# elizabethfong/SparkSmithWaterman

Hardware: AMD Instinct MI355X
Metric: GCUPS (higher is better)
Workload: dtype int32

## Files before the change

### sparksmithwaterman_amd/csrc/swmi_ctx.cpp

```cpp
#include <cstdarg>
#include <cstdio>
#include <cstdlib>

#include "swmi_host.h"
#include "swmi_launch.h"

static thread_local std::string g_err;

int swmi_host::fail(int code, const char *fmt, ...) {
    char buf[512];
    va_list ap;
    va_start(ap, fmt);
    vsnprintf(buf, sizeof buf, fmt, ap);
    va_end(ap);
    g_err = buf;
    return code;
}

int swmi_io_fail(int code, const std::string &msg) { return fail(code, "%s", msg.c_str()); }

extern "C" int swmi_abi_version(void) { return SWMI_ABI_VERSION; }

extern "C" const char *swmi_last_error(void) { return g_err.c_str(); }

// ... 108 lines not shown
    } else if (!strcmp(name, "resident")) {
        if (value < -1 || value > 1) return fail(SWMI_ERR_INVALID, "resident must be -1 (automatic), 0 or 1");
        ctx->resident = (int)value;
    } else if (!strcmp(name, "scores_only")) {
        ctx->scores_only = value != 0;
    } else if (!strcmp(name, "stream_keep_records")) {
        ctx->stream_keep_records = value != 0;
    } else if (!strcmp(name, "device_strings")) {
        ctx->device_strings = value != 0;
    } else if (!strcmp(name, "tb_split")) {
        if (value < -1 || value > 1) return fail(SWMI_ERR_INVALID, "tb_split must be -1 (automatic), 0 or 1");
        ctx->tb_split = (int)value;
    } else if (!strcmp(name, "col_chunks")) {
        if (value < 0 || value > 4096) return fail(SWMI_ERR_INVALID, "col_chunks out of range");
        ctx->col_chunks = (uint32_t)value;
    } else if (!strcmp(name, "zero_copy")) {
        ctx->zero_copy = value != 0;
    } else if (!strcmp(name, "profiling")) {
        if (value < 0 || value > 2) return fail(SWMI_ERR_INVALID, "profiling must be 0, 1 (every stage) or 2 (the sweep only)");
        ctx->profiling = (int)value;
    } else if (!strcmp(name, "gap_open")) {
        if (value > 0) return fail(SWMI_ERR_INVALID, "gap_open must be <= 0 (a penalty), got %lld", (long long)value);
        if (value < INT32_MIN) return fail(SWMI_ERR_INVALID, "gap_open out of range");
        ctx->gap_open = (int32_t)value;
    } else if (!strcmp(name, "affine")) {
        if (value != -1 && value != 1) return fail(SWMI_ERR_INVALID, "affine must be -1 (when gap_open != 0) or 1 (always)");
        ctx->affine = (int)value;
    } else if (!strcmp(name, "align_mode")) {
        if (value != SWMI_ALIGN_LOCAL && value != SWMI_ALIGN_FIT && value != SWMI_ALIGN_GLOBAL)
            return fail(SWMI_ERR_INVALID, "align_mode must be 0 (local), 1 (fit) or 2 (global), got %lld", (long long)value);
// ... 347 lines not shown
```

### sparksmithwaterman_amd/csrc/swmi_device.h

```cpp
#pragma once
#include <stdint.h>

#if defined(__HIPCC__)
#define SWMI_HD __host__ __device__
#else
#define SWMI_HD
#endif

#define SWMI_SEQ_PAD_WORDS 24u
#define SWMI_RMAX          4
#ifndef SWMI_CK_BLOCKS
#define SWMI_CK_BLOCKS     2u
#endif
#define SWMI_CODE_PAD      0x1FFu

#define SWMI_LDS_BYTES (160u * 1024u)
#define SWMI_EMIT_SCRATCH_WORDS 128u
#define SWMI_TB_BLOCKS 16u
#define SWMI_TB_REFWIN_WORDS 96u
#define SWMI_RES_CELL_CAP 128u

#define SWMI_DIR_D 0u
#define SWMI_DIR_I 1u
#define SWMI_DIR_A 2u
// ... 18 lines not shown
    uint32_t read_id;
    uint32_t out_id;
    uint32_t pad;
    uint64_t dir_off;
    uint64_t seam_off;
};

#define SWMI_PAD_COLS 0x80000000u
#define SWMI_PAD_RESIDENT 0x40000000u

struct ColItem {
    uint32_t pair;
    uint32_t col0;
    uint32_t g_lo, g_hi;
};

struct StripItem {
    uint32_t pair, strip;
    uint32_t col0, g_lo, g_hi;
    uint32_t prog;
    uint32_t priv_stride;
    uint32_t pad;
    uint64_t priv_off;
};

struct PairOut {
    int32_t  score;
    uint32_t flags;
    uint64_t n_cells;
};
// ... 232 lines not shown
```

### sparksmithwaterman_amd/csrc/swmi_host.h

```cpp
#pragma once
#include <hip/hip_runtime.h>

#include <algorithm>
#include <atomic>
#include <condition_variable>
#include <cstdint>
#include <cstring>
#include <memory>
#include <mutex>
#include <string>
#include <thread>
#include <type_traits>
#include <unordered_map>
#include <vector>

#include "../../include/swmi.h"
#include "swmi_device.h"
#include "swmi_io_internal.h"

namespace swmi_host __attribute__((visibility("hidden"))) {
int fail(int code, const char *fmt, ...);
int check_offsets(const uint64_t *off, uint32_t n, const char *what);
int upload_device(swmi_ctx *ctx, swmi_batch *b, hipStream_t st, const uint8_t *ref_src, const uint8_t *read_src);
int settle_raw(swmi_batch *b);
// ... 129 lines not shown
    uint64_t arena_words_per_pair = 160;
    uint64_t arena_copy_wpp = 160;
    uint64_t recs_per_pair_x16 = 32;
    hipEvent_t ev[6] = {nullptr, nullptr, nullptr, nullptr, nullptr, nullptr};
    PinnedBuf h_err;
    DevBuf d_hdr_ring;
    uint32_t hdr_next = 0;
    DevBuf d_lut;
    DevBuf d_comp;
    int64_t spin_us = 2000;
    uint32_t dbg_strip_spins = 0;
    uint32_t dbg_reverse_strips = 0;
    uint32_t dbg_async_delay_us = 0;
    uint32_t auto_ties_x100 = 300;
    uint32_t col_chunks = 0;
    int tb_split = -1;
    bool ext_events = false;
    int tfused = -1;
    int resident = -1;
    int scores_only = 0;
    int stream_keep_records = 1;
    int device_strings = 1;
    bool cell_cap_set = false;
    int32_t gap_open = 0;
    int affine = -1;
    RunModes modes;
    std::mutex mat_mu;
    std::shared_ptr<const ScoreMatrix> matrix;
    std::thread worker;
    std::mutex job_mu;
// ... 33 lines not shown

struct Work {
    uint32_t pair;
    uint64_t cells;
    uint64_t dir_words;
    uint64_t seam_words;
};

struct __attribute__((visibility("hidden"))) PlanKey {
    bool valid = false;
    size_t lo = 0, hi = 0;
    const void *work = nullptr;
    swmi_params params{};
    uint32_t eff_mode = 0;
    uint32_t col_chunks = 0;
    bool reverse_strips = false;
    int resident = -1, tfused = -1;
    bool exact = false;
    bool scores_only = false;
    uint64_t mat_gen = 0;
    RunModes modes;
    const void *d_pairs = nullptr;
    size_t pairs_bytes = 0;
    bool operator==(const PlanKey &o) const {
        return valid == o.valid && lo == o.lo && hi == o.hi && work == o.work && memcmp(&params, &o.params, sizeof(swmi_params)) == 0 &&
               eff_mode == o.eff_mode && col_chunks == o.col_chunks && reverse_strips == o.reverse_strips && resident == o.resident &&
               tfused == o.tfused && exact == o.exact && scores_only == o.scores_only && mat_gen == o.mat_gen &&
               modes == o.modes && d_pairs == o.d_pairs && pairs_bytes == o.pairs_bytes;
    }
};

struct __attribute__((visibility("hidden"))) ChunkPlan {
    uint64_t dir_words = 0, seam_words = 0;
    uint64_t seam_priv_words = 0;
    uint32_t max_path = 0, max_read = 0;
    size_t n_strip_items = 0;
    size_t n_strip_chunks = 0;
    size_t n_col_items = 0;
    uint64_t n_windows = 0;
    size_t n_res = 0;
    uint32_t res_lds_words = 0, res_ops_words = 0;
    size_t n_tf = 0;
    uint32_t tf_max_m = 0, tf_max_n = 0, tf_max_path = 0;
    uint32_t aff_r_min = 0xFFFFFFFFu, aff_r_max = 0;
    size_t aff_n_long = 0;
};

struct swmi_batch {
    uint32_t n_refs = 0, n_reads = 0;
    bool paired = false;
    uint32_t n_src_refs = 0, n_src_reads = 0;
    std::vector<swmi_pair_spec> specs;
    bool sources_on_device = false;
// ... 98 lines not shown
```

### sparksmithwaterman_amd/csrc/swmi_plan.h

```cpp
#pragma once
#include <chrono>
#include <cstdlib>

#include "swmi_host.h"

using Clock = std::chrono::steady_clock;
static inline double us_between(Clock::time_point a, Clock::time_point c) { return std::chrono::duration<double, std::micro>(c - a).count(); }

static uint64_t path_bound(uint64_t n_, uint64_t m_, const swmi_params &p, int32_t smax, int align_mode = 0) {
    uint64_t path = n_ + m_;
    if (align_mode != 0) return path;
    if (smax > 0 && p.gap < 0 && p.mismatch <= smax) {
        const uint64_t g = (uint64_t)(-(int64_t)p.gap), mt = (uint64_t)smax;
        path = std::min(path, std::min(m_ + std::min(n_, mt * m_ / g), n_ + std::min(m_, mt * n_ / g)));
    }
    return path;
}

static uint64_t traceback_lds_bytes(uint32_t mode, uint64_t max_path, uint64_t max_read) {
    const uint64_t lds_words = (max_path + 3) / 4 + 1, lds_read_words = (max_read + 3) / 4 + 1;
    const uint64_t win = (uint64_t)SWMI_RMAX * 64;
    const uint64_t tile_words = mode == 0 ? 4ull * SWMI_TB_BLOCKS * win : (mode == 1 ? 32 + 8ull * SWMI_CK_BLOCKS * win : 4ull * SWMI_CK_BLOCKS * win);
    return 4ull * (tile_words + 4ull * (lds_words + lds_read_words + SWMI_TB_REFWIN_WORDS));
}
// ... 32 lines not shown
    if (c.g_hi < n_ck && (uint64_t)c.g_hi * CK_STEP_W > n) c.g_hi = n_ck;
    const int64_t c0 = (int64_t)g_lo * CK_STEP_W - 64 - (int64_t)span - 1;
    c.col0 = g_lo == 0 || c0 <= 0 ? 0u : (uint32_t)(c0 / CK_STEP_W * CK_STEP_W);
    return c;
}

struct Planner {
    const swmi_ctx *ctx;
    const swmi_batch *b;
    const swmi_params &P;
    size_t np;
    ChunkPlan &plan;
    PlanItems &it;
    bool cols_possible = false;
    uint64_t chunk_budget = 1;
    bool res_possible = false, res_maybe = false;
    bool tf_possible = false;

    Planner(const swmi_ctx *ctx_, const swmi_batch *b_, size_t np_, bool exact, ChunkPlan &plan_, PlanItems &it_)
        : ctx(ctx_), b(b_), P(b_->params), np(np_), plan(plan_), it(it_) {
        const bool mode1 = b->eff_mode == 1, whole = mode1 && !exact && !ctx->scores_only;
        cols_possible = mode1 && P.match > 0 && P.gap < 0 && P.mismatch <= 0 && P.match <= 7 && P.mismatch >= -8 &&
                        (np <= 512 || ctx->col_chunks > 1) && ctx->col_chunks != 1;
        chunk_budget = ctx->col_chunks > 1 ? ctx->col_chunks : std::max<uint64_t>(1, 1024 / std::max<size_t>(np, 1));
        res_possible = whole && ctx->resident != 0 && (ctx->resident == 1 || np >= 256) &&
                       P.match <= 7 && P.match >= -8 && P.mismatch >= -8 && P.mismatch <= 0 && P.gap <= 0;
        tf_possible = whole && ctx->tfused == 1 &&
                      P.match > 0 && P.match <= 7 && P.mismatch >= -8 && P.mismatch <= P.match && P.gap < 0 && P.gap >= -64;
    }
    bool fast_symbols(const PairDesc &d) const { return b->read_desc[d.read_id].acgt && b->ref_desc[d.ref_id].acgt; }

    uint64_t res_need_words(uint32_t m, uint32_t n, uint32_t &opw) const {
        const uint32_t R_ = swmi_rows_per_lane(m), lact = (m + R_ - 1) / R_;
        const uint64_t nblk = ((uint64_t)n + lact - 1 + 15) / 16, n_ck = (nblk + SWMI_CK_BLOCKS - 1) / SWMI_CK_BLOCKS;
        opw = (uint32_t)((path_bound(n, m, P, P.match) + 15) / 16 + 1);
        return nblk * R_ * 64 + ((n_ck + 1) & ~1ull) + 2ull * SWMI_RES_CELL_CAP + 64ull * opw + (n + 3) / 4 + 1 + (m + 3) / 4 + 1 + 8 +
               SWMI_EMIT_SCRATCH_WORDS;
    }
// ... 71 lines not shown
        static const bool dbg_one = getenv("SWMI_DEBUG_ONE_CHUNK") != nullptr;
        if (dbg_one) chunks = 1;
        if (chunks < 2 && !dbg_one) return;
        const uint32_t wpc = (uint32_t)((n_ck + chunks - 1) / chunks);
        const size_t first = it.col_items.size();
        for (uint32_t g_lo = 0; g_lo < n_ck; g_lo += wpc) {
            const ColChunk c = col_chunk(g_lo, wpc, n_ck, n, span);
            ColItem ci;
            ci.pair = (uint32_t)k; ci.g_lo = c.g_lo; ci.g_hi = c.g_hi; ci.col0 = c.col0;
            it.col_items.push_back(ci);
            if (c.g_hi == n_ck) break;
        }
        d.pad = SWMI_PAD_COLS | (uint32_t)(it.col_items.size() - first);
    }

    void finish(const std::vector<Work> &work, size_t lo) {
        for (uint32_t k : it.res_items) {
            uint32_t opw;
            const uint64_t own = res_need_words(b->read_desc[it.pd[k].read_id].len, b->ref_desc[it.pd[k].ref_id].len, opw);
            plan.res_lds_words = std::max<uint32_t>(plan.res_lds_words, (uint32_t)(own + 64ull * (plan.res_ops_words - opw)));
        }
        if (16ull * plan.res_lds_words > SWMI_LDS_BYTES) {
            for (uint32_t k : it.res_items) it.pd[k].pad = 0;
            it.res_items.clear();
            plan.res_lds_words = 0; plan.res_ops_words = 0;
        }
        plan.n_strip_items = it.strip_items.size();
        plan.n_col_items = it.col_items.size();
        plan.n_res = it.res_items.size();
        plan.n_tf = it.tf_items.size();
        std::vector<uint8_t> is_res(np, 0);
        for (uint32_t k : it.res_items) is_res[k] = 1;
        for (size_t k = 0; k < np; k++) {
            it.pd[k].dir_off = plan.dir_words;
            it.pd[k].seam_off = plan.seam_words;
            if (!is_res[k]) { plan.dir_words += work[lo + k].dir_words; plan.seam_words += work[lo + k].seam_words; }
        }
        if (b->eff_mode == 1) it.win_off[np] = (uint32_t)std::min<uint64_t>(plan.n_windows, 0xFFFFFFFFu);
        for (StripItem &si : it.strip_items)
            if (si.priv_stride) si.priv_off += plan.seam_words;
    }
};

}

static int plan_chunk(swmi_ctx *ctx, swmi_batch *b, const std::vector<Work> &work, size_t lo, size_t np, bool exact, ChunkPlan &plan,
                      PlanItems &it) {
    plan = ChunkPlan{};
    Planner pl(ctx, b, np, exact, plan, it);
    if (pl.res_possible)
        for (size_t k = 0; k < np && !pl.res_maybe; k++)
            pl.res_maybe = pl.res_size_fits(b->read_desc[pair_read(b, work[lo + k].pair)].len, b->ref_desc[pair_ref(b, work[lo + k].pair)].len);
    if ((pl.cols_possible || pl.res_maybe || pl.tf_possible) && !b->acgt_known) {
        if (b->n_refs) HIP_TRY(hipMemcpy(b->ref_desc.data(), b->d_refs.p, b->n_refs * sizeof(SeqDesc), hipMemcpyDeviceToHost));
        if (b->n_reads) HIP_TRY(hipMemcpy(b->read_desc.data(), b->d_reads.p, b->n_reads * sizeof(SeqDesc), hipMemcpyDeviceToHost));
        b->acgt_known = true;
    }
    it.pd.resize(np);
    if (b->eff_mode == 1) it.win_off.resize(np + 1);
    uint32_t pb_m = 0xFFFFFFFFu, pb_n = 0xFFFFFFFFu, pb_val = 0;
    const int32_t smax = b->opt.mat ? std::max(b->params.match, b->opt.mat->max_entry) : b->params.match;
    for (size_t k = 0; k < np; k++) {
        const Work &w = work[lo + k];
        PairDesc d{};
        d.ref_id = pair_ref(b, w.pair);
        d.read_id = pair_read(b, w.pair);
        d.out_id = (uint32_t)k;
        const uint32_t m_ = b->read_desc[d.read_id].len, n_ = b->ref_desc[d.ref_id].len;
        if (b->eff_mode == 1) {
            const uint64_t rps = 64ull * swmi_rows_per_lane(m_);
            it.win_off[k] = (uint32_t)std::min<uint64_t>(plan.n_windows, 0xFFFFFFFFu);
            plan.n_windows += ((m_ + rps - 1) / rps) * ck_windows(n_);
        }
        const bool res_fit = pl.res_maybe && pl.fast_symbols(d) && pl.res_size_fits(m_, n_);
        if (!res_fit && pl.tf_fits(d, w, m_, n_)) pl.take_tfused(k, d, m_, n_);
        else if (res_fit) pl.take_resident(k, d, m_, n_);
        else if (b->eff_mode == 1 && m_ > 64u * SWMI_RMAX && it.strip_items.size() < (1u << 30)) pl.take_strips(k, d, m_, n_);
        else if (pl.cols_fit(d, m_)) pl.take_cols(k, d, m_, n_);
        it.pd[k] = d;
        if (m_ != pb_m || n_ != pb_n) { pb_m = m_; pb_n = n_; pb_val = (uint32_t)path_bound(n_, m_, b->params, smax, b->opt.modes.align_mode); }
        plan.max_path = std::max<uint32_t>(plan.max_path, pb_val);
        plan.max_read = std::max(plan.max_read, m_);
        if (m_ > SWMI_AFF_MAX_READ) { plan.aff_n_long++; continue; }
        plan.aff_r_min = std::min(plan.aff_r_min, swmi_aff_rows_per_lane(m_));
        plan.aff_r_max = std::max(plan.aff_r_max, swmi_aff_rows_per_lane(m_));
    }
    pl.finish(work, lo);
    if (b->eff_mode == 3 && plan.aff_n_long) {
        std::stable_partition(it.pd.begin(), it.pd.end(), [&](const PairDesc &d) { return b->read_desc[d.read_id].len <= SWMI_AFF_MAX_READ; });
    }
    return SWMI_OK;
}
// ... 27 lines not shown
        b->pairs_on_device.assign((const uint8_t *)it.pd.data(), (const uint8_t *)it.pd.data() + bytes);
        b->pairs_dev_ptr = b->d_pairs.p;
    }
    return SWMI_OK;
}

static int prepare_chunk(RunState &rs, const std::vector<Work> &work, size_t lo, size_t hi, const std::vector<uint64_t> *cells_exact) {
    swmi_ctx *ctx = rs.ctx;
    swmi_batch *b = rs.b;
    const size_t np = hi - lo;
    const auto p0 = Clock::now();
    PlanKey key;
    key.valid = true;
    key.lo = lo; key.hi = hi; key.work = (const void *)work.data();
    key.params = b->params; key.eff_mode = b->eff_mode;
    key.col_chunks = ctx->col_chunks; key.reverse_strips = ctx->dbg_reverse_strips != 0;
    key.resident = ctx->resident; key.tfused = ctx->tfused;
    key.exact = cells_exact != nullptr; key.scores_only = ctx->scores_only != 0;
    key.mat_gen = b->opt.mat ? b->opt.mat->gen : 0u; key.modes = b->opt.modes;
    key.d_pairs = b->d_pairs.p; key.pairs_bytes = np * sizeof(PairDesc);
    auto p1 = p0;
    if (key == b->plan_key) {
        p1 = Clock::now();
    } else {
        b->plan_key = PlanKey{};
        PlanItems items;
        int rc;
        if ((rc = plan_chunk(ctx, b, work, lo, np, key.exact, b->plan, items))) return rc;
        p1 = Clock::now();
        if ((rc = upload_plan(ctx, b, np, b->plan, items))) return rc;
        key.d_pairs = b->pairs_dev_ptr;
// ... 7 lines not shown
```

### sparksmithwaterman_amd/csrc/swmi_run.cpp

```cpp
#include <chrono>
#include <cstdio>
#include <cstdlib>
#include <functional>
#include <numeric>

#include "swmi_host.h"
#include "swmi_launch.h"
#include "swmi_plan.h"

static int keep_chunk_records(RunState &rs, const AlnRec *tab, uint64_t n_rec, const uint32_t *arena, uint64_t arena_cap, size_t lo) {
    swmi_batch *b = rs.b;
    if (rs.defer_copy && b->raw_chunks.empty()) {
        b->raw_ext = arena; b->rtab_ext = tab; b->raw_ext_records = n_rec; b->raw_ext_cap = arena_cap;
        b->raw_chunks.push_back(swmi_batch::RawChunk{0, 0, 0, (size_t)n_rec, lo, {}});
        return SWMI_OK;
    }
    uint64_t used = 0;
    for (uint64_t k = 0; k < n_rec; k++) {
        uint64_t end;
        if (!payload_end(b, tab[k], arena, arena_cap, end)) return fail(SWMI_ERR_HIP, "record payloads overrun the arena");
        used = std::max(used, end);
    }
    b->raw_chunks.push_back(swmi_batch::RawChunk{b->raw.size(), (size_t)used, b->rtab.size(), (size_t)n_rec, lo, {}});
    b->raw.insert(b->raw.end(), arena, arena + used);
// ... 85 lines not shown
    }
    fa.n_pairs = (uint32_t)L.np;
    fa.cell_cap = L.cell_cap;
    fa.match = b->params.match; fa.mismatch = b->params.mismatch; fa.gap = b->params.gap;
    fa.strict = b->params.tie_mode == SWMI_TIE_STRICT;
    fa.mode = b->eff_mode;
    const bool pipe = plan.n_strip_items && !rs.one_wave_sweep;
    fa.skip_multi = pipe ? 1u : 0u;
    fa.strip_items = pipe ? b->d_strip_items.as<StripItem>() : nullptr;
    fa.progress = pipe ? b->d_progress.as<uint32_t>() : nullptr;
    fa.n_strip_items = pipe ? (uint32_t)plan.n_strip_items : 0u;
    fa.err_host = (uint32_t *)ctx->h_err.dp;
    fa.n_out = (uint32_t)L.np;
    if (L.attempt == 0) b->timing.col_chunks += (uint32_t)plan.n_col_items + (pipe ? (uint32_t)plan.n_strip_chunks : 0u);
    fa.col_items = plan.n_col_items ? b->d_col_items.as<ColItem>() : nullptr;
    fa.n_col_items = (uint32_t)plan.n_col_items;
    fa.strip_spins = ctx->dbg_strip_spins;
    L.q_cap = std::min<uint64_t>(std::max<uint64_t>(L.cells_total, 1), 1ull << 24);
    if (L.split && (rc = b->d_queue.reserve(256 + L.q_cap * sizeof(uint4)))) return rc;
    fa.q_reset = L.split ? b->d_queue.as<uint32_t>() : nullptr;
    return SWMI_OK;
}

static int build_trace_args(RunState &rs, Launch &L) {
    swmi_ctx *ctx = rs.ctx;
    swmi_batch *b = rs.b;
    const ChunkPlan &plan = b->plan;
    const FillArgs &fa = rs.fa;
    int rc;
    TraceArgs &ta = rs.ta;
    ta.seqw = fa.seqw; ta.refs = fa.refs; ta.reads = fa.reads; ta.pairs = fa.pairs;
// ... 856 lines not shown
```

### sparksmithwaterman_amd/csrc/swmi_stream.cpp

```cpp
#include <chrono>
#include <cstdio>
#include <cstdlib>
#include <deque>

#include "swmi_host.h"

struct StreamChunk {
    uint32_t id = 0;
    PinnedBuf *buf = nullptr;
    std::vector<uint64_t> off;
    std::vector<swmi_io_recpos> recs;
    std::vector<uint8_t> keep;
};

struct swmi_stream {
    swmi_ctx *owner = nullptr;
    swmi_params params{};
    std::vector<uint8_t> read_bytes;
    std::vector<uint64_t> read_off;
    uint32_t n_reads = 0;
    uint64_t chunk_bytes = 32ull << 20;
    bool keep_records = true;
    struct Slot { swmi_ctx *ctx = nullptr; swmi_batch *shell = nullptr; std::thread th; };
    std::vector<Slot> slots;
// ... 129 lines not shown
    if (slots == 0) slots = 3;
    if (slots > 8) return fail(SWMI_ERR_INVALID, "at most 8 slots");
    std::unique_ptr<swmi_stream> s(new swmi_stream);
    s->owner = ctx;
    s->params = *p;
    s->n_reads = n_reads;
    s->read_off.assign(read_off, read_off + n_reads + 1);
    s->read_bytes.assign(read_bytes, read_bytes + read_off[n_reads]);
    if (chunk_bytes) s->chunk_bytes = std::max<uint64_t>(chunk_bytes, 1 << 16);
    s->keep_records = ctx->stream_keep_records != 0;
    s->slots.resize(slots);
    for (auto &sl : s->slots) {
        if ((rc = swmi_create(ctx->device, &sl.ctx))) { swmi_stream_close(s.release()); return rc; }
        sl.ctx->cell_cap = ctx->cell_cap; sl.ctx->cell_cap_set = ctx->cell_cap_set; sl.ctx->max_workspace_bytes = ctx->max_workspace_bytes;
        sl.ctx->profiling = ctx->profiling; sl.ctx->mode = ctx->mode; sl.ctx->zero_copy = ctx->zero_copy;
        sl.ctx->tb_split = ctx->tb_split; sl.ctx->col_chunks = ctx->col_chunks; sl.ctx->resident = ctx->resident; sl.ctx->tfused = ctx->tfused;
        sl.ctx->auto_ties_x100 = ctx->auto_ties_x100; sl.ctx->arena_words_per_pair = ctx->arena_words_per_pair;
        sl.ctx->device_strings = ctx->device_strings; sl.ctx->scores_only = ctx->scores_only;
        sl.ctx->gap_open = ctx->gap_open; sl.ctx->affine = ctx->affine;
        sl.ctx->modes = ctx->modes; sl.ctx->matrix = run_options(ctx).mat;
        sl.ctx->spin_us = 50;
        sl.shell = new swmi_batch;
    }
    const size_t n_bufs = slots + 8;
    for (size_t k = 0; k < n_bufs; k++) {
        std::unique_ptr<PinnedBuf> pb(new PinnedBuf);
        if ((rc = pb->reserve(s->chunk_bytes + (1 << 20)))) { swmi_stream_close(s.release()); return rc; }
        s->free_bufs.push_back(pb.get());
        s->bufs.push_back(std::move(pb));
    }
    for (size_t k = 0; k < s->slots.size(); k++) s->slots[k].th = std::thread(stream_worker, s.get(), k);
// ... 244 lines not shown
```

### sparksmithwaterman_amd/csrc/swmi_sweep.hip

```cpp
#include <hip/hip_runtime.h>
#include <hip/hip_ext.h>
#include <stdint.h>
#include <stdlib.h>
#include "swmi_device.h"
#include "swmi_launch.h"
#include "swmi_cells.h"

typedef uint32_t Words4 __attribute__((ext_vector_type(4)));
typedef const Words4 __attribute__((address_space(4))) *ConstWords4;

#define SWMI_PIPE_PUBLISH 2u
template <int R, bool ACGT, bool STRICT, bool MULTI, int MODE, bool PIPE = false>
__device__ __forceinline__ void fill_pair(const FillArgs &A, const PairDesc pd, const uint32_t lane, const uint32_t my_strip = 0u,
                                          const StripItem *item = nullptr) {
    const SeqDesc rd = A.refs[pd.ref_id];
    const SeqDesc qd = A.reads[pd.read_id];
    const uint32_t n_full = PIPE ? uni(rd.len) : rd.len, m = PIPE ? uni(qd.len) : qd.len;
    const uint32_t col0 = PIPE ? uni(item->col0) : 0u;
    const uint32_t g_lo = PIPE ? uni(item->g_lo) : 0u, g_hi = PIPE ? uni(item->g_hi) : 0xFFFFFFFFu;
    const uint32_t priv_stride = PIPE ? uni(item->priv_stride) : 0u;
    const uint32_t *__restrict__ refw = A.seqw + (PIPE ? uni(rd.boff) + (col0 >> 2) : rd.boff);
    const uint32_t *__restrict__ readw = A.seqw + qd.boff;
    const int match = A.match, mismatch = A.mismatch, gap = A.gap;
    constexpr uint32_t HMODE = MODE == SWMI_MODE_FIELD ? 0u : (MODE == SWMI_MODE_WINMAX ? 1u : 2u);
// ... 174 lines not shown
    if (lane == 0) {
        PairOut o;
        if (MODE == SWMI_MODE_WINMAX) {
            if (pair_max <= 0) { o.score = 0; o.flags = SWMI_F_DEGENERATE; o.n_cells = (uint64_t)m * n_full; }
            else               { o.score = pair_max; o.flags = 0u; o.n_cells = 0; }
        } else if (S.cnt == 0) { o.score = 0; o.flags = SWMI_F_DEGENERATE; o.n_cells = (uint64_t)m * n_full; }
        else            { o.score = S.thr; o.flags = S.cnt > ccap ? SWMI_F_CELL_OVF : 0u; o.n_cells = S.cnt; }
        A.out[pd.out_id] = o;
        if (A.dbg) {
            A.dbg[2 * pd.out_id] = S.events;
            A.dbg[2 * pd.out_id + 1] = __builtin_amdgcn_s_memtime() - t_start;
        }
    }
}

template <int R, bool COLS>
__device__ __forceinline__ void sweep_fast(const FillArgs &A, const PairDesc pd, const uint32_t lane, const ColItem ci) {
    const SeqDesc rd = A.refs[pd.ref_id];
    const SeqDesc qd = A.reads[pd.read_id];
    const uint32_t n_full = rd.len, m = qd.len;
    const StripGeom G = strip_geom<R>(m, n_full, 1u);
    const uint32_t col0 = COLS ? ci.col0 : 0u;
    const uint32_t g_lo = COLS ? ci.g_lo : 0u, g_hi = COLS ? ci.g_hi : G.n_ck;
    const bool last = g_hi >= G.n_ck;
    const uint32_t n = (last ? n_full : 16u * SWMI_CK_BLOCKS * g_hi) - col0;
    const uint32_t *__restrict__ refw = A.seqw + rd.boff + (col0 >> 2);
    const uint32_t *__restrict__ readw = A.seqw + qd.boff;
    const uint32_t lact = m >= G.rps ? WAVE : (m + R - 1) / R;
    const uint32_t lane_eff = lane < lact ? lane : 0x40000000u;
    const uint32_t T = n + lact - 1;
    const uint32_t nblk = last ? (T + 15u) / 16u : n / 16u;
    const uint32_t gm = (uint32_t)(-(int64_t)A.gap);
    const int one = 1;
    int pair_max = 0;

    const unsigned long long dbg_t0 = A.dbg ? __builtin_amdgcn_s_memtime() : 0ull;
    SweepState<R> S;
    build_profiles<R>(S.q, readw, lane * R, m, A.match, A.mismatch);
#pragma unroll
    for (int k = 0; k < R; ++k) {
// ... 11 lines not shown
        if (lane == 0) A.dir[pd.dir_off + G.wmax_off + g] = (uint32_t)wm;
        pair_max = pair_max > wm ? pair_max : wm;
        S.lmax = -1;
    };
    int steady_max = -1;
    bool closed = false;
    for (uint32_t tb = 0; tb < nblk; ++tb) {
        const uint32_t tbg = tb + (col0 >> 4);
        if ((tbg % SWMI_CK_BLOCKS) == 0u) {
            const uint32_t g = tbg / SWMI_CK_BLOCKS;
            if (tb > 0u && !closed) {
                if (g > g_lo) close_window(g - 1u); else S.lmax = -1;
            }
            closed = false;
#if !defined(SWMI_NO_ASM) && SWMI_CK_BLOCKS == 2u
            const uint32_t nwin = n > 16u * tb ? (n - 16u * tb) / 32u : 0u;
            if (g >= g_lo && nwin > 0u) {
                uint32_t cko = (g * (uint32_t)(R + 2) * WAVE + lane) * 4u;
                uint32_t wmo = ((uint32_t)G.wmax_off + g - 1u) * 4u;
                uint32_t rfo = tb * 16u;
                const uint32_t lact_s = uni(lact);
                int wm_last;
                uint32_t wx = wnext.x, wy = wnext.y, wz = wnext.z, ww = wnext.w;
                SweepWindowAsm<R>::run(S.h, S.g, S.hp, S.q, S.rbx, S.rby, wx, wy, wz, ww, one, gm, S.lmax, wm_last, steady_max,
                                       cko, wmo, rfo, uni64((uint64_t)(uintptr_t)(A.dir + pd.dir_off)), uni64((uint64_t)(uintptr_t)refq),
                                       lact_s >= WAVE ? ~0ull : (1ull << lact_s) - 1ull, uni(nwin - 1u));
                wnext = make_uint4(wx, wy, wz, ww);
                const int wm = wave_max_i32(wm_last);
                if (lane == 0) A.dir[pd.dir_off + G.wmax_off + g + nwin - 1u] = (uint32_t)wm;
                tb += 2u * nwin - 1u;
                closed = true;
                continue;
            }
#endif
            if (g >= g_lo) {
                uint32_t *__restrict__ ck = wsp + (uint64_t)g * (R + 2) * WAVE;
#pragma unroll
                for (int k = 0; k < R; ++k) ck[k * WAVE] = (uint32_t)S.h[k];
                ck[R * WAVE] = (uint32_t)wave_shr1_zero(S.g[R - 1]);
                ck[(R + 1) * WAVE] = (uint32_t)S.rby;
            }
        }
        const uint4 w = wnext;
        wnext = refq[tb + 1];
// ... 6 lines not shown
            SweepStep4Asm<R>::run(S.h, S.g, S.hp, S.q, S.rbx, S.rby, w.w, wnext.x, one, gm, S.lmax);
        } else
#endif
        {
            sweep_tail_block<R>(S, w, wnext.x, t0, lane_eff, n, one, gm);
        }
    }
    if (!closed) {
        const uint32_t gl = (nblk - 1u + (col0 >> 4)) / SWMI_CK_BLOCKS;
        if (gl >= g_lo) close_window(gl);
    }
    {
        const int sm = wave_max_i32(steady_max);
        pair_max = pair_max > sm ? pair_max : sm;
    }
    if (lane != 0) return;
    if (A.dbg) {
        A.dbg[2 * pd.out_id] = (unsigned long long)__builtin_amdgcn_s_getreg((4 ) | (0 << 6) | (31 << 11)) |
                               ((unsigned long long)__builtin_amdgcn_s_getreg((20 ) | (0 << 6) | (31 << 11)) << 32);
        A.dbg[2 * pd.out_id + 1] = __builtin_amdgcn_s_memtime() - dbg_t0;
    }
    PairOut *o = &A.out[pd.out_id];
    if (COLS) {
        if (pair_max > 0) atomicMax(&o->score, pair_max);
        return;
    }
    PairOut v;
    if (pair_max <= 0) { v.score = 0; v.flags = SWMI_F_DEGENERATE; v.n_cells = (uint64_t)m * n_full; }
    else               { v.score = pair_max; v.flags = 0u; v.n_cells = 0; }
    *o = v;
}

template <bool COLS>
__device__ __forceinline__ void sweep_fast_dispatch(const FillArgs &A, const PairDesc pd, uint32_t lane, uint32_t m, const ColItem ci) {
    const uint32_t R = swmi_rows_per_lane(m);
    if (R == 1)      sweep_fast<1, COLS>(A, pd, lane, ci);
    else if (R == 2) sweep_fast<2, COLS>(A, pd, lane, ci);
    else if (R == 3) sweep_fast<3, COLS>(A, pd, lane, ci);
    else             sweep_fast<4, COLS>(A, pd, lane, ci);
}

template <bool ACGT, bool STRICT, int MODE>
__device__ __forceinline__ void fill_dispatch(const FillArgs &A, const PairDesc pd, uint32_t lane, uint32_t m) {
    const uint32_t R = swmi_rows_per_lane(m);
    if (R == 1)      fill_pair<1, ACGT, STRICT, false, MODE>(A, pd, lane);
    else if (R == 2) fill_pair<2, ACGT, STRICT, false, MODE>(A, pd, lane);
    else if (R == 3) fill_pair<3, ACGT, STRICT, false, MODE>(A, pd, lane);
    else if (m <= WAVE * SWMI_RMAX) fill_pair<SWMI_RMAX, ACGT, STRICT, false, MODE>(A, pd, lane);
    else             fill_pair<SWMI_RMAX, ACGT, STRICT, true, MODE>(A, pd, lane);
}

template <int MODE>
__device__ __forceinline__ void fill_entry(const FillArgs &A) {
    const uint32_t pair = blockIdx.x * FILL_WAVES + (threadIdx.x >> 6);
// ... 54 lines not shown
    const uint32_t strip = __builtin_amdgcn_readfirstlane(it->strip);
    if (acgt) fill_pair<SWMI_RMAX, true, false, true, SWMI_MODE_WINMAX, true>(A, pd, lane, strip, it);
    else      fill_pair<SWMI_RMAX, false, false, true, SWMI_MODE_WINMAX, true>(A, pd, lane, strip, it);
}

extern "C" __global__ void __launch_bounds__(WAVE * FILL_WAVES)
sw_sweep_winmax_cols_kernel(const FillArgs A) {
    const uint32_t item = blockIdx.x * FILL_WAVES + (threadIdx.x >> 6);
    if (item >= A.n_col_items) return;
    const uint32_t lane = threadIdx.x & 63u;
    const ColItem ci = A.col_items[item];
    const PairDesc pd = A.pairs[ci.pair];
    sweep_fast_dispatch<true>(A, pd, lane, A.reads[pd.read_id].len, ci);
}

static size_t spread_lds(uint32_t n_groups) {
    static const int on = getenv("SWMI_LDS_SPREAD") ? atoi(getenv("SWMI_LDS_SPREAD")) : 1;
    if (!on || n_groups == 0 || n_groups > 4u * 256u) return 0;
    const uint32_t per_cu = (n_groups + 255u) / 256u;
    return ((size_t)(160u * 1024u) / (per_cu + 1u) / 1024u + 1u) * 1024u;
}

extern "C" hipError_t swmi_launch_fill(const FillArgs *a, hipStream_t st, hipEvent_t ev_start, hipEvent_t ev_stop) {
    if (a->n_pairs == 0) return hipSuccess;
    static const bool attrs = [] {
        swmi_allow_big_lds(sw_fill_kernel); swmi_allow_big_lds(sw_fill_score_kernel); swmi_allow_big_lds(sw_sweep_winmax_kernel);
        swmi_allow_big_lds(sw_sweep_winmax_strips_kernel); swmi_allow_big_lds(sw_sweep_winmax_cols_kernel);
        return true;
    }();
    (void)attrs;
    const dim3 grid((a->n_pairs + FILL_WAVES - 1) / FILL_WAVES), block(WAVE * FILL_WAVES);
    const size_t lds = spread_lds(grid.x);
    if (a->mode == 0)      hipLaunchKernelGGL(sw_fill_kernel, grid, block, lds, st, *a);
    else if (a->mode == 1) {
        if (ev_start && ev_stop && !(a->skip_multi && a->n_strip_items) && !a->n_col_items) {
            hipExtLaunchKernelGGL(sw_sweep_winmax_kernel, grid, block, (uint32_t)lds, st, ev_start, ev_stop, 0u, *a);
            return hipGetLastError();
        }
        hipLaunchKernelGGL(sw_sweep_winmax_kernel, grid, block, a->n_col_items || a->n_strip_items ? 0 : lds, st, *a);
        if (a->skip_multi && a->n_strip_items) {
            const uint32_t g = (a->n_strip_items + FILL_WAVES - 1) / FILL_WAVES;
            hipLaunchKernelGGL(sw_sweep_winmax_strips_kernel, dim3(g), block, spread_lds(g), st, *a);
        }
        if (a->n_col_items) {
            const uint32_t g = (a->n_col_items + FILL_WAVES - 1) / FILL_WAVES;
            hipLaunchKernelGGL(sw_sweep_winmax_cols_kernel, dim3(g), block, spread_lds(g), st, *a);
        }
    }
    else                   hipLaunchKernelGGL(sw_fill_score_kernel, grid, block, lds, st, *a);
    return hipGetLastError();
}
```

Measured before the change: 2554.

## Split each alignment into two cooperating column halves synchronized through LDS

Adds a paired column mode in which each pair's reference is split into a left and right half, each swept by a sibling wave in the same workgroup. The right wave publishes checkpoints over a halo region. The left wave runs past its boundary, compares its state against those checkpoints and stops once they converge. The max scores are then combined through LDS atomics. This is meant to double parallelism when there are too few pairs to fill the GPU (about 512 pairs), and the default heuristic enables it automatically. The cost is halo recomputation, spin-waiting and a new kernel path.

New measurement: 2510. 1.7% lower.

```diff
diff --git a/sparksmithwaterman_amd/csrc/swmi_ctx.cpp b/sparksmithwaterman_amd/csrc/swmi_ctx.cpp
--- a/sparksmithwaterman_amd/csrc/swmi_ctx.cpp
+++ b/sparksmithwaterman_amd/csrc/swmi_ctx.cpp
@@ -146,6 +146,9 @@
     } else if (!strcmp(name, "col_chunks")) {
         if (value < 0 || value > 4096) return fail(SWMI_ERR_INVALID, "col_chunks out of range");
         ctx->col_chunks = (uint32_t)value;
+    } else if (!strcmp(name, "col_pairing")) {
+        if (value < -1 || value > 1) return fail(SWMI_ERR_INVALID, "col_pairing must be -1 (automatic), 0 or 1");
+        ctx->col_pairing = (int)value;
     } else if (!strcmp(name, "zero_copy")) {
         ctx->zero_copy = value != 0;
     } else if (!strcmp(name, "profiling")) {
diff --git a/sparksmithwaterman_amd/csrc/swmi_device.h b/sparksmithwaterman_amd/csrc/swmi_device.h
--- a/sparksmithwaterman_amd/csrc/swmi_device.h
+++ b/sparksmithwaterman_amd/csrc/swmi_device.h
@@ -56,6 +56,13 @@
     uint32_t col0;
     uint32_t g_lo, g_hi;
 };
+#define SWMI_COLS_PAIRED      0x80000000u
+#define SWMI_COLS_PAIRED_ONLY 0x40000000u
+#define SWMI_COLS_COUNT(n)    ((n) & 0x3FFFFFFFu)
+static inline SWMI_HD uint32_t swmi_pair_halo_windows(uint32_t m, int32_t match, int32_t gap) {
+    const uint32_t span = m + (uint32_t)match * m / (uint32_t)(-gap) + 1u;
+    return (span + 64u + 31u) / 32u;
+}
 
 struct StripItem {
     uint32_t pair, strip;
diff --git a/sparksmithwaterman_amd/csrc/swmi_host.h b/sparksmithwaterman_amd/csrc/swmi_host.h
--- a/sparksmithwaterman_amd/csrc/swmi_host.h
+++ b/sparksmithwaterman_amd/csrc/swmi_host.h
@@ -167,6 +167,7 @@
     uint32_t dbg_async_delay_us = 0;
     uint32_t auto_ties_x100 = 300;
     uint32_t col_chunks = 0;
+    int col_pairing = -1;
     int tb_split = -1;
     bool ext_events = false;
     int tfused = -1;
@@ -230,6 +231,7 @@
     swmi_params params{};
     uint32_t eff_mode = 0;
     uint32_t col_chunks = 0;
+    int col_pairing = -1;
     bool reverse_strips = false;
     int resident = -1, tfused = -1;
     bool exact = false;
@@ -240,7 +242,7 @@
     size_t pairs_bytes = 0;
     bool operator==(const PlanKey &o) const {
         return valid == o.valid && lo == o.lo && hi == o.hi && work == o.work && memcmp(&params, &o.params, sizeof(swmi_params)) == 0 &&
-               eff_mode == o.eff_mode && col_chunks == o.col_chunks && reverse_strips == o.reverse_strips && resident == o.resident &&
+               eff_mode == o.eff_mode && col_chunks == o.col_chunks && col_pairing == o.col_pairing && reverse_strips == o.reverse_strips && resident == o.resident &&
                tfused == o.tfused && exact == o.exact && scores_only == o.scores_only && mat_gen == o.mat_gen &&
                modes == o.modes && d_pairs == o.d_pairs && pairs_bytes == o.pairs_bytes;
     }
@@ -253,6 +255,7 @@
     size_t n_strip_items = 0;
     size_t n_strip_chunks = 0;
     size_t n_col_items = 0;
+    uint32_t col_paired = 0;
     uint64_t n_windows = 0;
     size_t n_res = 0;
     uint32_t res_lds_words = 0, res_ops_words = 0;
diff --git a/sparksmithwaterman_amd/csrc/swmi_plan.h b/sparksmithwaterman_amd/csrc/swmi_plan.h
--- a/sparksmithwaterman_amd/csrc/swmi_plan.h
+++ b/sparksmithwaterman_amd/csrc/swmi_plan.h
@@ -70,6 +70,7 @@
     PlanItems &it;
     bool cols_possible = false;
     uint64_t chunk_budget = 1;
+    bool pairing = false;
     bool res_possible = false, res_maybe = false;
     bool tf_possible = false;
 
@@ -78,6 +79,8 @@
         const bool mode1 = b->eff_mode == 1, whole = mode1 && !exact && !ctx->scores_only;
         cols_possible = mode1 && P.match > 0 && P.gap < 0 && P.mismatch <= 0 && P.match <= 7 && P.mismatch >= -8 &&
                         (np <= 512 || ctx->col_chunks > 1) && ctx->col_chunks != 1;
+        pairing = mode1 && SWMI_CK_BLOCKS == 2u && P.match > 0 && P.gap < 0 && P.mismatch <= 0 && P.match <= 7 && P.mismatch >= -8 &&
+                  (ctx->col_pairing == 1 || (ctx->col_pairing < 0 && ctx->col_chunks == 0 && np <= 512 && 1024 / std::max<size_t>(np, 1) == 2));
         chunk_budget = ctx->col_chunks > 1 ? ctx->col_chunks : std::max<uint64_t>(1, 1024 / std::max<size_t>(np, 1));
         res_possible = whole && ctx->resident != 0 && (ctx->resident == 1 || np >= 256) &&
                        P.match <= 7 && P.match >= -8 && P.mismatch >= -8 && P.mismatch <= 0 && P.gap <= 0;
@@ -179,6 +182,24 @@
         d.pad = SWMI_PAD_COLS | (uint32_t)(it.col_items.size() - first);
     }
 
+    bool take_pairing(size_t k, PairDesc &d, uint32_t m, uint32_t n) {
+        if (!pairing || m > 64u * SWMI_RMAX || !fast_symbols(d)) return false;
+        const uint32_t halo_w = swmi_pair_halo_windows(m, P.match, P.gap), n_steady = n / CK_STEP_W;
+        if (n_steady < 2u * halo_w) return false;
+        const uint32_t R_ = swmi_rows_per_lane(m), lact = (m + R_ - 1) / R_;
+        const uint32_t windows = (n + lact - 1 + CK_STEP_W - 1) / CK_STEP_W;
+        const uint32_t ov = (uint32_t)((path_span(m, P) / 2 + 64 + CK_STEP_W - 1) / CK_STEP_W);
+        uint32_t g_split = windows > ov ? (windows - ov + 1) / 2 : 0;
+        g_split = std::min(std::max(g_split, halo_w), n_steady - halo_w);
+        ColItem left, right;
+        left.pair = (uint32_t)k; left.col0 = 0; left.g_lo = 0; left.g_hi = g_split;
+        right.pair = (uint32_t)k; right.col0 = g_split * CK_STEP_W; right.g_lo = g_split; right.g_hi = ck_windows(n);
+        it.col_items.push_back(left);
+        it.col_items.push_back(right);
+        d.pad = SWMI_PAD_COLS | 2u;
+        return true;
+    }
+
     void finish(const std::vector<Work> &work, size_t lo) {
         for (uint32_t k : it.res_items) {
             uint32_t opw;
@@ -192,6 +213,7 @@
         }
         plan.n_strip_items = it.strip_items.size();
         plan.n_col_items = it.col_items.size();
+        if (pairing && plan.n_col_items) plan.col_paired = plan.n_col_items == 2 * np ? 2u : 1u;
         plan.n_res = it.res_items.size();
         plan.n_tf = it.tf_items.size();
         std::vector<uint8_t> is_res(np, 0);
@@ -216,7 +238,7 @@
     if (pl.res_possible)
         for (size_t k = 0; k < np && !pl.res_maybe; k++)
             pl.res_maybe = pl.res_size_fits(b->read_desc[pair_read(b, work[lo + k].pair)].len, b->ref_desc[pair_ref(b, work[lo + k].pair)].len);
-    if ((pl.cols_possible || pl.res_maybe || pl.tf_possible) && !b->acgt_known) {
+    if ((pl.cols_possible || pl.pairing || pl.res_maybe || pl.tf_possible) && !b->acgt_known) {
         if (b->n_refs) HIP_TRY(hipMemcpy(b->ref_desc.data(), b->d_refs.p, b->n_refs * sizeof(SeqDesc), hipMemcpyDeviceToHost));
         if (b->n_reads) HIP_TRY(hipMemcpy(b->read_desc.data(), b->d_reads.p, b->n_reads * sizeof(SeqDesc), hipMemcpyDeviceToHost));
         b->acgt_known = true;
@@ -241,6 +263,7 @@
         if (!res_fit && pl.tf_fits(d, w, m_, n_)) pl.take_tfused(k, d, m_, n_);
         else if (res_fit) pl.take_resident(k, d, m_, n_);
         else if (b->eff_mode == 1 && m_ > 64u * SWMI_RMAX && it.strip_items.size() < (1u << 30)) pl.take_strips(k, d, m_, n_);
+        else if (pl.pairing) (void)pl.take_pairing(k, d, m_, n_);
         else if (pl.cols_fit(d, m_)) pl.take_cols(k, d, m_, n_);
         it.pd[k] = d;
         if (m_ != pb_m || n_ != pb_n) { pb_m = m_; pb_n = n_; pb_val = (uint32_t)path_bound(n_, m_, b->params, smax, b->opt.modes.align_mode); }
@@ -298,7 +321,7 @@
     key.valid = true;
     key.lo = lo; key.hi = hi; key.work = (const void *)work.data();
     key.params = b->params; key.eff_mode = b->eff_mode;
-    key.col_chunks = ctx->col_chunks; key.reverse_strips = ctx->dbg_reverse_strips != 0;
+    key.col_chunks = ctx->col_chunks; key.col_pairing = ctx->col_pairing; key.reverse_strips = ctx->dbg_reverse_strips != 0;
     key.resident = ctx->resident; key.tfused = ctx->tfused;
     key.exact = cells_exact != nullptr; key.scores_only = ctx->scores_only != 0;
     key.mat_gen = b->opt.mat ? b->opt.mat->gen : 0u; key.modes = b->opt.modes;
diff --git a/sparksmithwaterman_amd/csrc/swmi_run.cpp b/sparksmithwaterman_amd/csrc/swmi_run.cpp
--- a/sparksmithwaterman_amd/csrc/swmi_run.cpp
+++ b/sparksmithwaterman_amd/csrc/swmi_run.cpp
@@ -123,7 +123,7 @@
     fa.n_out = (uint32_t)L.np;
     if (L.attempt == 0) b->timing.col_chunks += (uint32_t)plan.n_col_items + (pipe ? (uint32_t)plan.n_strip_chunks : 0u);
     fa.col_items = plan.n_col_items ? b->d_col_items.as<ColItem>() : nullptr;
-    fa.n_col_items = (uint32_t)plan.n_col_items;
+    fa.n_col_items = (uint32_t)plan.n_col_items | (plan.col_paired ? SWMI_COLS_PAIRED : 0u) | (plan.col_paired == 2u ? SWMI_COLS_PAIRED_ONLY : 0u);
     fa.strip_spins = ctx->dbg_strip_spins;
     L.q_cap = std::min<uint64_t>(std::max<uint64_t>(L.cells_total, 1), 1ull << 24);
     if (L.split && (rc = b->d_queue.reserve(256 + L.q_cap * sizeof(uint4)))) return rc;
diff --git a/sparksmithwaterman_amd/csrc/swmi_stream.cpp b/sparksmithwaterman_amd/csrc/swmi_stream.cpp
--- a/sparksmithwaterman_amd/csrc/swmi_stream.cpp
+++ b/sparksmithwaterman_amd/csrc/swmi_stream.cpp
@@ -167,7 +167,7 @@
         if ((rc = swmi_create(ctx->device, &sl.ctx))) { swmi_stream_close(s.release()); return rc; }
         sl.ctx->cell_cap = ctx->cell_cap; sl.ctx->cell_cap_set = ctx->cell_cap_set; sl.ctx->max_workspace_bytes = ctx->max_workspace_bytes;
         sl.ctx->profiling = ctx->profiling; sl.ctx->mode = ctx->mode; sl.ctx->zero_copy = ctx->zero_copy;
-        sl.ctx->tb_split = ctx->tb_split; sl.ctx->col_chunks = ctx->col_chunks; sl.ctx->resident = ctx->resident; sl.ctx->tfused = ctx->tfused;
+        sl.ctx->tb_split = ctx->tb_split; sl.ctx->col_chunks = ctx->col_chunks; sl.ctx->col_pairing = ctx->col_pairing; sl.ctx->resident = ctx->resident; sl.ctx->tfused = ctx->tfused;
         sl.ctx->auto_ties_x100 = ctx->auto_ties_x100; sl.ctx->arena_words_per_pair = ctx->arena_words_per_pair;
         sl.ctx->device_strings = ctx->device_strings; sl.ctx->scores_only = ctx->scores_only;
         sl.ctx->gap_open = ctx->gap_open; sl.ctx->affine = ctx->affine;
diff --git a/sparksmithwaterman_amd/csrc/swmi_sweep.hip b/sparksmithwaterman_amd/csrc/swmi_sweep.hip
--- a/sparksmithwaterman_amd/csrc/swmi_sweep.hip
+++ b/sparksmithwaterman_amd/csrc/swmi_sweep.hip
@@ -212,8 +212,9 @@
     }
 }
 
-template <int R, bool COLS>
-__device__ __forceinline__ void sweep_fast(const FillArgs &A, const PairDesc pd, const uint32_t lane, const ColItem ci) {
+template <int R, bool COLS, int PAIRED = 0>
+__device__ __forceinline__ void sweep_fast(const FillArgs &A, const PairDesc pd, const uint32_t lane, const ColItem ci,
+                                           uint32_t *sync = nullptr) {
     const SeqDesc rd = A.refs[pd.ref_id];
     const SeqDesc qd = A.reads[pd.read_id];
     const uint32_t n_full = rd.len, m = qd.len;
@@ -221,7 +222,13 @@
     const uint32_t col0 = COLS ? ci.col0 : 0u;
     const uint32_t g_lo = COLS ? ci.g_lo : 0u, g_hi = COLS ? ci.g_hi : G.n_ck;
     const bool last = g_hi >= G.n_ck;
-    const uint32_t n = (last ? n_full : 16u * SWMI_CK_BLOCKS * g_hi) - col0;
+    const uint32_t halo_w = PAIRED ? swmi_pair_halo_windows(m, A.match, A.gap) : 0u;
+    const uint32_t g_stop = PAIRED == 1 ? (g_hi + halo_w < n_full / 32u ? g_hi + halo_w : n_full / 32u) : g_hi;
+    const uint32_t n = (last ? n_full : 16u * SWMI_CK_BLOCKS * g_stop) - col0;
+    uint32_t published = 0u;
+    uint32_t seen = 0u, rck_v[R + 2];
+    bool rck_ahead = false;
+    (void)published; (void)seen; (void)rck_v; (void)rck_ahead;
     const uint32_t *__restrict__ refw = A.seqw + rd.boff + (col0 >> 2);
     const uint32_t *__restrict__ readw = A.seqw + qd.boff;
     const uint32_t lact = m >= G.rps ? WAVE : (m + R - 1) / R;
@@ -263,7 +270,38 @@
             }
             closed = false;
 #if !defined(SWMI_NO_ASM) && SWMI_CK_BLOCKS == 2u
-            const uint32_t nwin = n > 16u * tb ? (n - 16u * tb) / 32u : 0u;
+            uint32_t nwin = n > 16u * tb ? (n - 16u * tb) / 32u : 0u;
+            if (PAIRED == 1) {
+                if (g < g_hi) nwin = g_hi - g;
+                else {
+                    while (seen < g - g_hi + 1u) {
+                        seen = __hip_atomic_load(sync, __ATOMIC_ACQUIRE, __HIP_MEMORY_SCOPE_WORKGROUP);
+                        if (seen < g - g_hi + 1u) __builtin_amdgcn_s_sleep(2);
+                    }
+                    const uint32_t *rck = wsp + (uint64_t)g * (R + 2) * WAVE;
+                    if (!rck_ahead) {
+#pragma unroll
+                        for (int k = 0; k < R + 2; ++k) rck_v[k] = __hip_atomic_load(rck + k * WAVE, __ATOMIC_RELAXED, __HIP_MEMORY_SCOPE_WORKGROUP);
+                    }
+                    bool differs = false;
+#pragma unroll
+                    for (int k = 0; k < R; ++k) differs |= rck_v[k] != (uint32_t)S.h[k];
+                    differs |= rck_v[R] != (uint32_t)wave_shr1_zero(S.g[R - 1]);
+                    differs |= rck_v[R + 1] != (uint32_t)S.rby;
+                    if (__ballot(differs && lane < lact) == 0ull) {
+                        closed = true;
+                        break;
+                    }
+                    nwin = 1u;
+                    rck_ahead = seen >= g - g_hi + 2u;
+                    if (rck_ahead) {
+#pragma unroll
+                        for (int k = 0; k < R + 2; ++k)
+                            rck_v[k] = __hip_atomic_load(rck + (R + 2) * WAVE + k * WAVE, __ATOMIC_RELAXED, __HIP_MEMORY_SCOPE_WORKGROUP);
+                    }
+                }
+            }
+            if (PAIRED == 2 && published < halo_w && nwin > 1u) nwin = 1u;
             if (g >= g_lo && nwin > 0u) {
                 uint32_t cko = (g * (uint32_t)(R + 2) * WAVE + lane) * 4u;
                 uint32_t wmo = ((uint32_t)G.wmax_off + g - 1u) * 4u;
@@ -275,8 +313,16 @@
                                        cko, wmo, rfo, uni64((uint64_t)(uintptr_t)(A.dir + pd.dir_off)), uni64((uint64_t)(uintptr_t)refq),
                                        lact_s >= WAVE ? ~0ull : (1ull << lact_s) - 1ull, uni(nwin - 1u));
                 wnext = make_uint4(wx, wy, wz, ww);
+                const bool announce = PAIRED == 2 && published < halo_w;
+                if (announce && published > 0u) {
+                    if (lane == 0) __hip_atomic_store(sync, published, __ATOMIC_RELEASE, __HIP_MEMORY_SCOPE_WORKGROUP);
+                }
                 const int wm = wave_max_i32(wm_last);
                 if (lane == 0) A.dir[pd.dir_off + G.wmax_off + g + nwin - 1u] = (uint32_t)wm;
+                if (announce && ++published == halo_w) {
+                    asm volatile("s_waitcnt vmcnt(0)" ::: "memory");
+                    if (lane == 0) __hip_atomic_store(sync, published, __ATOMIC_RELEASE, __HIP_MEMORY_SCOPE_WORKGROUP);
+                }
                 tb += 2u * nwin - 1u;
                 closed = true;
                 continue;
@@ -313,6 +359,10 @@
         const int sm = wave_max_i32(steady_max);
         pair_max = pair_max > sm ? pair_max : sm;
     }
+    if (PAIRED == 2) {
+        asm volatile("s_waitcnt vmcnt(0)" ::: "memory");
+        if (lane == 0) __hip_atomic_store(sync, 0xFFFFFFFFu, __ATOMIC_RELEASE, __HIP_MEMORY_SCOPE_WORKGROUP);
+    }
     if (lane != 0) return;
     if (A.dbg) {
         A.dbg[2 * pd.out_id] = (unsigned long long)__builtin_amdgcn_s_getreg((4 ) | (0 << 6) | (31 << 11)) |
@@ -320,6 +370,12 @@
         A.dbg[2 * pd.out_id + 1] = __builtin_amdgcn_s_memtime() - dbg_t0;
     }
     PairOut *o = &A.out[pd.out_id];
+    if (PAIRED) {
+        __hip_atomic_store(sync + 1 + PAIRED, (uint32_t)pair_max, __ATOMIC_RELAXED, __HIP_MEMORY_SCOPE_WORKGROUP);
+        if (__hip_atomic_fetch_add(sync + 1, 1u, __ATOMIC_ACQ_REL, __HIP_MEMORY_SCOPE_WORKGROUP) == 0u) return;
+        const int other = (int)__hip_atomic_load(sync + 4 - PAIRED, __ATOMIC_RELAXED, __HIP_MEMORY_SCOPE_WORKGROUP);
+        pair_max = pair_max > other ? pair_max : other;
+    } else
     if (COLS) {
         if (pair_max > 0) atomicMax(&o->score, pair_max);
         return;
@@ -330,13 +386,14 @@
     *o = v;
 }
 
-template <bool COLS>
-__device__ __forceinline__ void sweep_fast_dispatch(const FillArgs &A, const PairDesc pd, uint32_t lane, uint32_t m, const ColItem ci) {
+template <bool COLS, int PAIRED = 0>
+__device__ __forceinline__ void sweep_fast_dispatch(const FillArgs &A, const PairDesc pd, uint32_t lane, uint32_t m, const ColItem ci,
+                                                    uint32_t *sync = nullptr) {
     const uint32_t R = swmi_rows_per_lane(m);
-    if (R == 1)      sweep_fast<1, COLS>(A, pd, lane, ci);
-    else if (R == 2) sweep_fast<2, COLS>(A, pd, lane, ci);
-    else if (R == 3) sweep_fast<3, COLS>(A, pd, lane, ci);
-    else             sweep_fast<4, COLS>(A, pd, lane, ci);
+    if (R == 1)      sweep_fast<1, COLS, PAIRED>(A, pd, lane, ci, sync);
+    else if (R == 2) sweep_fast<2, COLS, PAIRED>(A, pd, lane, ci, sync);
+    else if (R == 3) sweep_fast<3, COLS, PAIRED>(A, pd, lane, ci, sync);
+    else             sweep_fast<4, COLS, PAIRED>(A, pd, lane, ci, sync);
 }
 
 template <bool ACGT, bool STRICT, int MODE>
@@ -421,6 +478,26 @@
     sweep_fast_dispatch<true>(A, pd, lane, A.reads[pd.read_id].len, ci);
 }
 
+extern "C" __global__ void __launch_bounds__(WAVE * FILL_WAVES)
+sw_sweep_winmax_pairs_kernel(const FillArgs A) {
+#if !defined(SWMI_NO_ASM) && SWMI_CK_BLOCKS == 2u
+    __shared__ uint32_t sync[FILL_WAVES / 2][4];
+    if (threadIdx.x < 2u * FILL_WAVES) (&sync[0][0])[threadIdx.x] = 0u;
+    __syncthreads();
+    const uint32_t wave = threadIdx.x >> 6, item = blockIdx.x * FILL_WAVES + wave;
+    if (item >= SWMI_COLS_COUNT(A.n_col_items)) return;
+    const uint32_t lane = threadIdx.x & 63u;
+    if (item == 0 && lane == 0 && (A.n_col_items & SWMI_COLS_PAIRED_ONLY)) {
+        if (A.hdr) { A.hdr->reserved = 0; A.hdr->pad = 0; }
+        if (A.q_reset) *A.q_reset = 0u;
+    }
+    const ColItem ci = A.col_items[item];
+    const PairDesc pd = A.pairs[ci.pair];
+    if (wave & 1u) sweep_fast_dispatch<true, 2>(A, pd, lane, A.reads[pd.read_id].len, ci, sync[wave >> 1]);
+    else           sweep_fast_dispatch<true, 1>(A, pd, lane, A.reads[pd.read_id].len, ci, sync[wave >> 1]);
+#endif
+}
+
 static size_t spread_lds(uint32_t n_groups) {
     static const int on = getenv("SWMI_LDS_SPREAD") ? atoi(getenv("SWMI_LDS_SPREAD")) : 1;
     if (!on || n_groups == 0 || n_groups > 4u * 256u) return 0;
@@ -433,6 +510,7 @@
     static const bool attrs = [] {
         swmi_allow_big_lds(sw_fill_kernel); swmi_allow_big_lds(sw_fill_score_kernel); swmi_allow_big_lds(sw_sweep_winmax_kernel);
         swmi_allow_big_lds(sw_sweep_winmax_strips_kernel); swmi_allow_big_lds(sw_sweep_winmax_cols_kernel);
+        (void)hipFuncSetAttribute(reinterpret_cast<const void *>(sw_sweep_winmax_pairs_kernel), hipFuncAttributeMaxDynamicSharedMemorySize, 159 * 1024);
         return true;
     }();
     (void)attrs;
@@ -444,14 +522,26 @@
             hipExtLaunchKernelGGL(sw_sweep_winmax_kernel, grid, block, (uint32_t)lds, st, ev_start, ev_stop, 0u, *a);
             return hipGetLastError();
         }
+        const uint32_t n_cols = SWMI_COLS_COUNT(a->n_col_items);
+        if (a->n_col_items & SWMI_COLS_PAIRED) {
+#if defined(SWMI_NO_ASM) || SWMI_CK_BLOCKS != 2u
+            return hipErrorInvalidValue;
+#endif
+            if (a->n_col_items & SWMI_COLS_PAIRED_ONLY) {
+                const uint32_t g = (n_cols + FILL_WAVES - 1) / FILL_WAVES;
+                hipLaunchKernelGGL(sw_sweep_winmax_pairs_kernel, dim3(g), block, spread_lds(g), st, *a);
+                return hipGetLastError();
+            }
+        }
         hipLaunchKernelGGL(sw_sweep_winmax_kernel, grid, block, a->n_col_items || a->n_strip_items ? 0 : lds, st, *a);
         if (a->skip_multi && a->n_strip_items) {
             const uint32_t g = (a->n_strip_items + FILL_WAVES - 1) / FILL_WAVES;
             hipLaunchKernelGGL(sw_sweep_winmax_strips_kernel, dim3(g), block, spread_lds(g), st, *a);
         }
-        if (a->n_col_items) {
-            const uint32_t g = (a->n_col_items + FILL_WAVES - 1) / FILL_WAVES;
-            hipLaunchKernelGGL(sw_sweep_winmax_cols_kernel, dim3(g), block, spread_lds(g), st, *a);
+        if (n_cols) {
+            const uint32_t g = (n_cols + FILL_WAVES - 1) / FILL_WAVES;
+            if (a->n_col_items & SWMI_COLS_PAIRED) hipLaunchKernelGGL(sw_sweep_winmax_pairs_kernel, dim3(g), block, spread_lds(g), st, *a);
+            else               hipLaunchKernelGGL(sw_sweep_winmax_cols_kernel, dim3(g), block, spread_lds(g), st, *a);
         }
     }
     else                   hipLaunchKernelGGL(sw_fill_score_kernel, grid, block, lds, st, *a);
```
